# soedinglab/metaeuk

Hardware: AMD Instinct MI355X
Metric: prefilter+align ORF-fragments/sec (hits UNVERIFIED in this run: no CPU reference digest) (higher is better)
Workload: dtype packed i16 / i32 DP on u8 residues, i8 scores

## Files before the change

metaeuk_amd/csrc/mk_align.hip:

```cpp
#include "mk_align.hpp"
#include "mk_filters.hpp"
#include "mk_kernels.hpp"
#include "mk_segsort.hpp"
#include <algorithm>
#include <cmath>
#include <cstdlib>
#include <cstring>
#include <atomic>
#include <map>
#include <mutex>
#include <omp.h>

namespace mk {

namespace {

constexpr uint32_t KEY_CLS = 4096;
constexpr int SW_NBINCFG = SW_NCFG + 2;
constexpr uint32_t N_BINS = (uint32_t) SW_NBINCFG * KEY_CLS;
static_assert(SW_NCFG <= 16, "the bounds arrays keep 16 slots per kind");

__device__ __forceinline__ uint32_t len_class(uint32_t tLen) { return KEY_CLS - 1 - min(tLen >> 4, KEY_CLS - 1); }
__device__ __forceinline__ uint32_t sort_key(uint32_t qLen, uint32_t tLen) { return (uint32_t) sw_cfg_of(qLen) * KEY_CLS + len_class(tLen); }

// ... 461 lines not shown
        for (size_t k = 0; k < lens.size(); k++)
            if (!cached[k]) (*rowCache)[lens[k]].assign(&t.evalue[k * t.smax], &t.evalue[k * t.smax] + t.smax);
    if (t.bitScore.empty()) {
        t.bitScore.resize(32768);
        for (int s = 0; s < 32768; s++) t.bitScore[s] = static_cast<int>(ev.bitScore((double) s) + 0.5);
    }
}

void build_gate_table(const Evaluer &ev, double evalThr, const std::vector<uint64_t> &qOff, std::vector<GateEntry> &table, const AssembleTables *T) {
    uint32_t maxLen = 0;
    const size_t n = qOff.size() - 1;
    for (size_t i = 0; i < n; i++) maxLen = std::max<uint32_t>(maxLen, (uint32_t) (qOff[i + 1] - qOff[i]));
    std::vector<uint8_t> present(maxLen + 1, 0);
    for (size_t i = 0; i < n; i++) present[qOff[i + 1] - qOff[i]] = 1;
    table.assign(maxLen + 1, GateEntry{1 << 30, {0, 0, 0, 0, 0, 0, 0, 0}});
#pragma omp parallel for schedule(dynamic, 16)
    for (uint32_t L = 1; L <= maxLen; L++) {
        if (!present[L]) continue;
        GateEntry g;
        std::memset(&g, 0, sizeof(g));
        const int SCAN = 4096;
        const double *row = (T && L < T->lenIdx.size() && T->lenIdx[L] >= 0) ? T->evalue.data() + (size_t) T->lenIdx[L] * T->smax : nullptr;
        const auto eval = [&](int s) { return (row && (uint32_t) s < T->smax) ? row[s] : ev.evalue((double) s, (double) L); };
        int lastFail = 0;
        for (int s = SCAN; s >= 1; s--) {
            const bool pass = !(eval(s) > evalThr);
            if (!pass) { lastFail = s; break; }
        }
        g.s0 = lastFail >= SCAN ? (1 << 30) : lastFail + 1;
        for (int s = 1; s < 256 && s < g.s0; s++)
            if (!(eval(s) > evalThr)) g.mask[s >> 5] |= 1u << (s & 31);
        table[L] = g;
    }
}

#define ACHK(x) do { hipError_t e_ = (x); if (e_ != hipSuccess) { err = std::string(#x) + ": " + hipGetErrorString(e_); return MK_ERR_DEVICE; } } while (0)
#define ANULL(p) do { if (!(p)) { err = "device scratch allocation failed (" #p ")"; return MK_ERR_DEVICE; } } while (0)

static int device_scan(const uint32_t *in, uint32_t n, uint32_t *out, uint32_t *total, hipStream_t stream, std::string &err) {
    if (n == 0) { if (total) ACHK(hipMemsetAsync(total, 0, 4, stream)); return MK_OK; }
    const uint32_t nb = (n + SCAN_TILE - 1u) / SCAN_TILE;
    uint32_t *sums = (uint32_t *) dev_scratch("align_scansums", (size_t) nb * 4);
    ANULL(sums);
    hipLaunchKernelGGL(scan_sums_kernel, dim3(nb), dim3(256), 0, stream, in, n, sums);
    hipLaunchKernelGGL(scan_apply_kernel, dim3(nb), dim3(256), 0, stream, in, n, out, (const uint32_t *) sums, total);
    ACHK(hipGetLastError());
    return MK_OK;
}

struct AlignShapes {
    int cus = 256;
    uint32_t persistentBlocks[SW_NCFG];
    uint32_t unitsPerBlock = 0;
    int knownForce = -1, knownWaves = 12;
    bool fwdLargeFirst = false;
    bool multiLargeFirst = true;
    bool multiPrio = true;
    uint32_t multiPerCu[3] = {24, 12, 12};
};
static bool sw_early_exit() { return knob_long("MK_SW_EARLY_EXIT", 1) != 0; }
static const AlignShapes &align_shapes() {
    static AlignShapes S;
    static std::once_flag once;
    std::call_once(once, [] {
        int dev = 0;
        (void) hipGetDevice(&dev);
        if (hipDeviceGetAttribute(&S.cus, hipDeviceAttributeMultiprocessorCount, dev) != hipSuccess || S.cus <= 0) S.cus = 256;
        int perCu[SW_NCFG];
        for (int c = 0; c < SW_NCFG; c++) perCu[c] = 12;
        if (const char *e = knob("MK_SW_WAVES_PER_CU")) {
            int k = 0, last = 16;
            for (const char *p = e; *p && k < SW_NCFG; k++) {
                last = std::max(1, atoi(p));
                perCu[k] = last;
                while (*p && *p != ',') p++;
                if (*p == ',') p++;
            }
            for (; k < SW_NCFG; k++) perCu[k] = last;
        }
        for (int c = 0; c < SW_NCFG; c++) S.persistentBlocks[c] = (uint32_t) (S.cus * perCu[c]);
        S.unitsPerBlock = (uint32_t) std::max(0L, knob_long("MK_SW_UNITS_PER_BLOCK", 0));
        S.knownForce = (int) knob_long("MK_SW_KNOWN", -1);
        S.knownWaves = (int) std::max(1L, knob_long("MK_SW_KNOWN_WAVES", 12));
        S.multiPrio = knob_long("MK_SW_MULTI_PRIO", 1) != 0;
        S.fwdLargeFirst = knob_long("MK_SW_FWD_LARGE_FIRST", 0) != 0;
        S.multiLargeFirst = knob_long("MK_SW_MULTI_LARGE_FIRST", 1) != 0;
        if (const char *e = knob("MK_SW_MULTI_WAVES")) {
            int k = 0;
            for (const char *p = e; *p && k < 3; k++) { S.multiPerCu[k] = (uint32_t) std::max(1, atoi(p)); while (*p && *p != ',') p++; if (*p == ',') p++; }
        }
    });
    return S;
}

static int tpos_first_cfg(const AlignView &V) {
    static_assert(SW_NCFG == 11, "configurations 8 / 9 = 512 / 768 rows");
    if (!V.q_prof || knob_long("MK_SW_TPOS", 1) == 0 || knob_long("MK_SW_MULTI", 0) != 0 || knob_long("MK_SW_NARROW", -1) == 0) return -1;
    return 8;
}

static int run_sorted_sw(const AlignView &V, const mk_params &P, const SwJob *jobs, SwOut *out, const uint32_t *keys, uint32_t *hist, uint32_t *order,
                         uint32_t n, const char *tag, hipStream_t stream, std::string &err,
                         timed_begin_fn tb, timed_end_fn te, int *handles ,
                         const int32_t *knownScore ) {
    if (handles) for (int c = 0; c < SW_NCFG; c++) handles[c] = -1;
    if (n == 0) return MK_OK;
    const AlignShapes &S = align_shapes();
    uint32_t *dCursor = (uint32_t *) dev_scratch("align_bincursor", (size_t) N_BINS * 4);
    uint32_t *dBounds = (uint32_t *) dev_scratch("align_bounds", 64 * sizeof(uint32_t));
    uint32_t *hb = (uint32_t *) pinned_scratch("align_bounds_h", 64 * sizeof(uint32_t));
    ANULL(dCursor); ANULL(dBounds); ANULL(hb);
    int th = tb("align_sort", 12.0 * n, 0);
    hipLaunchKernelGGL(bin_scan_kernel, dim3(1), dim3(BIN_THREADS), 0, stream, hist, dCursor, dBounds);
    hipLaunchKernelGGL(bin_scatter_kernel, dim3((n + 255) / 256), dim3(256), 0, stream, keys, n, dCursor, order);
    te(th);
    ACHK(hipGetLastError());
    const bool knownPreferred = knownScore && !V.q_prof && (S.knownForce >= 0 ? S.knownForce != 0 : !V.co_resident);
    const bool multiLaunch = knob_long("MK_SW_MULTI", 0) != 0;
    if (multiLaunch && !knownPreferred && V.max_q_len <= (uint32_t) sw_cfg_rows(SW_NCFG - 1)) {
        uint32_t *dCnt = (uint32_t *) dev_scratch("align_multicounters", 64);
        ANULL(dCnt);
        ACHK(hipMemsetAsync(dCnt, 0, 64, stream));
        SwLaunch L;
        L.q_res = V.q_res; L.q_bias8 = V.q_bias8; L.q_prof = V.q_prof; L.t_res = V.t_res; L.mat = V.mat_aln;
        L.jobs = jobs; L.out = out; L.n_jobs = n; L.order = order;
        L.boundary = nullptr; L.boundary_stride = 0; L.boundary_job0 = 0;
        L.wave_start = nullptr; L.n_waves = 0; L.work_counter = nullptr; L.persistent_blocks = 0; L.units_per_block = 0;
        L.known_score = sw_early_exit() ? knownScore : nullptr;
        L.gap_open = P.gap_open; L.gap_extend = P.gap_extend;
        static const char *clsName[3] = {"rows32_64", "rows96_256", "rows384_1024"};
        static const int clsFirst[3] = {0, 3, 7};
        for (int kk = 0; kk < 3; kk++) {
            const int k = S.multiLargeFirst ? 2 - kk : kk;
            char nm[64];
            snprintf(nm, sizeof(nm), "%s_%s", tag, clsName[k]);
            th = tb(nm, 0, 0);
            if (handles) handles[clsFirst[k]] = th;
            const uint32_t units = (n + 3u) / 4u + (uint32_t) SW_NCFG;
            ACHK(launch_sw_multi(L, dBounds, dCnt + k, k, std::min(units, (uint32_t) S.cus * S.multiPerCu[k]), stream, S.multiPrio));
            te(th);
        }
        return MK_OK;
    }
    ACHK(hipMemcpyAsync(hb, dBounds, 64 * sizeof(uint32_t), hipMemcpyDeviceToHost, stream));
    ACHK(sync_wait(stream, "wait_align"));
    for (int c = 0; c < SW_NCFG; c++) {
        const uint32_t lo = hb[c], hi = hb[c + 1];
        if (hi <= lo) continue;
        SwLaunch L;
        L.q_res = V.q_res; L.q_bias8 = V.q_bias8; L.q_prof = V.q_prof; L.t_res = V.t_res; L.mat = V.mat_aln;
        L.jobs = jobs; L.out = out; L.n_jobs = hi - lo; L.order = order + lo;
        L.boundary = nullptr; L.boundary_stride = 0; L.boundary_job0 = 0;
        L.wave_start = nullptr; L.n_waves = 0; L.work_counter = nullptr; L.persistent_blocks = 0; L.units_per_block = 0; L.known_score = nullptr;
        L.gap_open = P.gap_open; L.gap_extend = P.gap_extend;
        if (c == SW_NCFG - 1 && V.max_q_len > (uint32_t) sw_cfg_rows(c)) {
            const uint32_t cls = KEY_CLS - 1 - (hb[32 + c] % KEY_CLS);
            const uint32_t stride = std::min<uint32_t>(V.max_t_len, (cls + 1) * 16);
            L.boundary = (uint32_t *) dev_scratch("align_border", (size_t) (hi - lo) * stride * sizeof(uint32_t));
            ANULL(L.boundary);
            L.boundary_stride = stride;
        }
        char nm[64];
        snprintf(nm, sizeof(nm), "%s_rows%d", tag, sw_cfg_rows(c));
        th = tb(nm, 0, 0);
        if (handles) handles[c] = th;
        if (knownScore && sw_cfg_known(c) && !V.q_prof && (S.knownForce >= 0 ? S.knownForce != 0 : !V.co_resident)) {
            uint32_t *dWork = (uint32_t *) dev_scratch("align_knowncounters", 64 * sizeof(uint32_t));
            ANULL(dWork);
            uint32_t *counter = dWork + (strcmp(tag, "sw_rev") == 0 ? 16 : 0) + c;
            ACHK(hipMemsetAsync(counter, 0, sizeof(uint32_t), stream));
            L.known_score = knownScore; L.work_counter = counter;
            L.persistent_blocks = (uint32_t) S.cus * (uint32_t) (sw_cfg_rows(c) <= 32 ? S.knownWaves : std::max(1, S.knownWaves / 2));
            ACHK(launch_sw_known(L, c, stream));
        } else {
            if (sw_early_exit()) L.known_score = knownScore;
            ACHK(launch_sw(L, c, stream));
        }
        te(th);
    }
    for (int pc = 0; pc < SW_NBINCFG - SW_NCFG; pc++) {
        const uint32_t lo = hb[SW_NCFG + pc], hi = hb[SW_NCFG + pc + 1];
        if (hi <= lo) continue;
        if (!knownScore || !V.q_prof) { err = "transposed position jobs without a known score"; return MK_ERR_DEVICE; }
        SwLaunch L;
        L.q_res = V.q_res; L.q_bias8 = V.q_bias8; L.q_prof = V.q_prof; L.t_res = V.t_res; L.mat = V.mat_aln;
        L.jobs = jobs; L.out = out; L.n_jobs = hi - lo; L.order = order + lo;
        L.boundary = nullptr; L.boundary_stride = 0; L.boundary_job0 = 0;
        L.wave_start = nullptr; L.n_waves = 0; L.work_counter = nullptr; L.persistent_blocks = 0; L.units_per_block = 0; L.known_score = knownScore;
        L.gap_open = P.gap_open; L.gap_extend = P.gap_extend;
        const int rows = sw_cfg_rows(8 + pc);
        char nm[64];
        snprintf(nm, sizeof(nm), "%s_rows%dt", tag, rows);
        th = tb(nm, 0, 0);
        ACHK(launch_sw_tpos(L, rows, (uint32_t) S.cus * (uint32_t) std::max(1L, knob_long("MK_SW_TPOS_WAVES", 32)), stream));
        te(th);
    }
    return MK_OK;
}

static int run_shared_fwd(const AlignView &V, const mk_params &P, const uint64_t *dHitOff, const mk_hit *dHits, const SwJob *jobs, SwOut *out,
                          uint32_t n, hipStream_t stream, std::string &err, timed_begin_fn tb, timed_end_fn te, int *handles ) {
    for (int c = 0; c < SW_NCFG; c++) handles[c] = -1;
    if (n == 0) return MK_OK;
    const AlignShapes &S = align_shapes();
    const uint32_t nq = V.n_queries;
    const uint32_t nb = (nq + PLAN_BLOCK - 1u) / PLAN_BLOCK;
    const uint32_t maxRuns = n / ORDER_TILE + nq + 1;
    uint32_t *dOrder = (uint32_t *) dev_scratch("align_order", (size_t) n * 4);
    uint32_t *dWave = (uint32_t *) dev_scratch("align_wavestart", ((size_t) n + 1) * 4);
    uint32_t *dPlan = (uint32_t *) dev_scratch("align_plan", ((size_t) nq * 2 + (size_t) maxRuns * 2 + (size_t) nb * (PLAN_NV + 1)) * 4);
    uint32_t *dBounds = (uint32_t *) dev_scratch("align_bounds", 64 * sizeof(uint32_t));
    uint32_t *hb = (uint32_t *) pinned_scratch("align_bounds_h", 64 * sizeof(uint32_t));
    uint32_t *dWork = (uint32_t *) dev_scratch("align_workcounters", 256);
    ANULL(dOrder); ANULL(dWave); ANULL(dPlan); ANULL(dBounds); ANULL(hb); ANULL(dWork);
    ACHK(hipMemsetAsync(dWork, 0, 256, stream));
    const long narrowForce = knob_long("MK_SW_NARROW", -1);
    const bool narrow = narrowForce >= 0 ? narrowForce != 0 : V.q_prof != nullptr;
    PlanArgs A;
    A.hitOff = dHitOff; A.q_off = V.q_off; A.nq = nq; A.nPairs = n; A.narrow = narrow;
    A.jobOff = dPlan; A.waveOff = dPlan + nq; A.runQuery = dPlan + 2 * (size_t) nq; A.runIndex = A.runQuery + maxRuns; A.blockSums = A.runIndex + maxRuns;
    A.bounds = dBounds; A.waveStart = dWave;
    int th = tb("align_sort", 24.0 * n, 0);
    hipLaunchKernelGGL(plan_sums_kernel, dim3(nb), dim3(PLAN_BLOCK), 0, stream, A);
    hipLaunchKernelGGL(plan_offsets_kernel, dim3(nb), dim3(PLAN_BLOCK), 0, stream, A);
    ACHK(hipGetLastError());
    ACHK(hipMemcpyAsync(hb, dBounds, 64 * sizeof(uint32_t), hipMemcpyDeviceToHost, stream));
// ... 407 lines not shown
```

metaeuk_amd/csrc/mk_kernels.hpp:

```cpp
#pragma once
#include <hip/hip_runtime.h>
#include <cstdint>

namespace mk {

struct SwJob {
    uint64_t t_start;
    uint32_t q_start;
    uint32_t q_len;
    uint32_t t_len;
    int32_t q_step;
    int32_t t_step;
    uint32_t slot;
};
struct SwOut { int32_t score; int32_t end_col; int32_t end_row; int32_t pad; };

struct SwLaunch {
    const uint8_t *q_res; const int8_t *q_bias8;
    const int8_t *q_prof = nullptr;
    const uint8_t *t_res;
    const int8_t *mat;
    const SwJob *jobs; SwOut *out; uint64_t n_jobs;
    const uint32_t *order;
    uint32_t *boundary;
    uint32_t boundary_stride;
    int gap_open, gap_extend;
    const uint32_t *wave_start; uint64_t n_waves;
    uint32_t *work_counter;
    uint32_t *work_counter_t = nullptr;
    uint32_t t_max_rows = 0;
    uint32_t persistent_blocks;
    uint32_t units_per_block;
    uint64_t boundary_job0;
    const int32_t *known_score;
    bool narrow = false;
};

constexpr int SW_NCFG = 11;
__host__ __device__ inline int sw_cfg_rows(int c) {
    const int rows[SW_NCFG] = {32, 48, 64, 96, 128, 192, 256, 384, 512, 768, 1024};
    return rows[c];
}
__host__ __device__ inline bool sw_cfg_packed(int c) { return sw_cfg_rows(c) <= 768; }
__host__ __device__ inline uint32_t sw_cfg_jobs_per_wave(int c, bool narrow = false) {
    const int rows = sw_cfg_rows(c);
    return rows <= 256 ? 8u : (rows <= 768 ? (narrow ? 8u : 4u) : 1u);
}
__host__ __device__ inline int sw_cfg_of(uint32_t qLen) {
    int c = 0;
    while (c < SW_NCFG - 1 && (uint32_t) sw_cfg_rows(c) < qLen) c++;
    return c;
}
hipError_t launch_sw(const SwLaunch &L, int cfg, hipStream_t stream);
hipError_t launch_sw_score(const SwLaunch &L, int cfg, hipStream_t stream);
__host__ __device__ inline bool sw_cfg_known(int c) { return sw_cfg_rows(c) <= 64; }
hipError_t launch_sw_known(const SwLaunch &L, int cfg, hipStream_t stream);
constexpr uint32_t SW_TPOS_MAX_ROWS = 256;
hipError_t launch_sw_tpos(const SwLaunch &L, int rows, uint32_t blocksPerClass, hipStream_t stream);
hipError_t launch_sw_multi(const SwLaunch &L, const uint32_t *bounds, uint32_t *counter, int cls, uint32_t blocks, hipStream_t stream, bool prio = true);

template <class ScoreFn>
__host__ __device__ inline int ungapped_on_diagonal_fn(ScoreFn score_of, uint32_t qLen, const uint8_t *t, uint32_t tLen,
                                                       int diagonal, uint32_t minDist) {
    uint32_t len = 0, q0 = 0, t0 = 0;
    if (diagonal >= 0 && minDist < qLen) { len = tLen < qLen - minDist ? tLen : qLen - minDist; q0 = minDist; }
    else if (diagonal < 0 && minDist < tLen) { len = tLen - minDist < qLen ? tLen - minDist : qLen; t0 = minDist; }
    int score = 0, best = 0;
    for (uint32_t k = 0; k < len; k++) {
        const int curr = score_of(q0 + k, (uint32_t) t[t0 + k]);
        score = score + curr > 0 ? score + curr : 0;
        best = best > score ? best : score;
    }
    return best;
}
template <class ScoreFn>
__host__ __device__ inline int ungapped_score_fn(ScoreFn score_of, uint32_t qLen, const uint8_t *t, uint32_t tLen, uint32_t d16) {
    if (qLen >= 32768u || tLen >= 32768u) {
        int best = 0;
        for (uint32_t d = 1; d <= 1u + tLen / 32768u; d++) {
            const int real = (int) (0u - d * 65536u + d16);
            const int m = ungapped_on_diagonal_fn(score_of, qLen, t, tLen, real, (uint32_t) (real < 0 ? -real : real));
            best = best > m ? best : m;
        }
        for (uint32_t d = 0; d <= qLen / 65536u; d++) {
            const int real = (int) (d * 65536u + d16);
            const int m = ungapped_on_diagonal_fn(score_of, qLen, t, tLen, real, (uint32_t) (real < 0 ? -real : real));
            best = best > m ? best : m;
        }
        return best;
    }
    const uint32_t dist = ((0x10000u - d16) & 0xFFFFu) < d16 ? ((0x10000u - d16) & 0xFFFFu) : d16;
    return ungapped_on_diagonal_fn(score_of, qLen, t, tLen, (int) (short) (uint16_t) d16, dist);
}
template <typename MatT>
__host__ __device__ inline int ungapped_score(const MatT *smat, const uint8_t *q, const int8_t *corr, uint32_t qLen, const uint8_t *t, uint32_t tLen, uint32_t d16) {
    return ungapped_score_fn([=](uint32_t i, uint32_t tr) -> int { return (int) (int8_t) ((int8_t) smat[q[i] * 21 + tr] + corr[i]); }, qLen, t, tLen, d16);
}
__host__ __device__ inline int ungapped_score_profile(const int8_t *aln, uint32_t qLen, const uint8_t *t, uint32_t tLen, uint32_t d16) {
    return ungapped_score_fn([=](uint32_t i, uint32_t tr) -> int { return (int) aln[(size_t) i * 32 + tr]; }, qLen, t, tLen, d16);
}

struct UngappedJob { uint64_t t_start; uint32_t q_start; uint32_t q_len; uint32_t t_len; uint32_t diagonal; };
struct UngappedLaunch {
    const uint8_t *q_res; const int8_t *q_corr;
    const uint8_t *t_masked;
    const int8_t *mat;
    const UngappedJob *jobs; int32_t *out; uint64_t n_jobs;
};
hipError_t launch_ungapped(const UngappedLaunch &L, hipStream_t stream);
// ... 36 lines not shown
```

metaeuk_amd/csrc/mk_sw.hip:

```cpp
#include "mk_kernels.hpp"
#include <algorithm>
#include <mutex>

namespace mk {

template <int G>
__device__ __forceinline__ uint32_t shift_up(uint32_t top, uint32_t x, int laneInGroup) {
    if constexpr (G == 16) {
        return (uint32_t) __builtin_amdgcn_update_dpp((int) top, (int) x, 0x111 , 0xf, 0xf, false);
    } else if constexpr (G == 64) {
        return (uint32_t) __builtin_amdgcn_update_dpp((int) top, (int) x, 0x138 , 0xf, 0xf, false);
    } else {
        const uint32_t v = (uint32_t) __builtin_amdgcn_update_dpp((int) top, (int) x, 0x138 , 0xf, 0xf, false);
        return laneInGroup == 0 ? top : v;
    }
}

template <int G>
__device__ __forceinline__ uint32_t shift_up_zero(uint32_t x, int laneInGroup) {
    if constexpr (G == 16) return (uint32_t) __builtin_amdgcn_update_dpp((int) x, (int) x, 0x111 , 0xf, 0xf, true);
    else return shift_up<G>(0u, x, laneInGroup);
}

__device__ __forceinline__ int max3i(int a, int b, int c) { return max(max(a, b), c); }
// ... 71 lines not shown
                const int q = row0 + row;
                const bool real = q < qLen;
                const int64_t qi = (int64_t) profQStart + (int64_t) (real ? q : 0) * profQStep;
                sQ[row] = real ? L.q_res[qi] : (uint8_t) 255;
                sB[row] = real ? L.q_bias8[qi] : (int8_t) 0;
            }
            __builtin_amdgcn_fence(__ATOMIC_ACQ_REL, "wavefront");
            __builtin_amdgcn_wave_barrier();
            for (int idx = SHARED ? (int) threadIdx.x : lane; idx < 22 * ROWS; idx += SHARED ? BLOCK : G) {
                const int t = idx / ROWS, row = idx - t * ROWS;
                const uint32_t qc = sQ[row];
                prof[idx] = (t < 21 && qc != 255u) ? (int8_t) ((int) sMat[t * 21 + (int) qc] + (int) sB[row]) : (int8_t) 0;
            }
        }
        __builtin_amdgcn_fence(__ATOMIC_ACQ_REL, "wavefront");
        __builtin_amdgcn_wave_barrier();

        int H[R], E[R];
        uint32_t key[R];
#pragma unroll
        for (int r = 0; r < R; r++) { H[r] = 0; E[r] = 0; key[r] = 0; }
        uint32_t out0 = 0, out1 = 21u;
        int hupPrev = 0;
        const int steps = tLen > 0 ? tLen + G - 1 : 0;
        const bool readTop = (tile > 0);
        const bool writeBottom = (tile + 1 < nTiles);
        const int laneRow = (int) (threadIdx.x & 15u);
        const int64_t tBase = (int64_t) job.t_start;
        const int64_t tStep = (int64_t) job.t_step;
        const int tLast = max(tLen - 1, 0);
        uint32_t tq0 = L.t_res[tBase + (int64_t) min(laneRow, tLast) * tStep], tq1 = L.t_res[tBase + (int64_t) min(16 + laneRow, tLast) * tStep],
                 tq2 = L.t_res[tBase + (int64_t) min(32 + laneRow, tLast) * tStep];
        for (int s0 = 0; s0 < steps; s0 += 16) {
            uint32_t tcur = tq0;
            tq0 = tq1; tq1 = tq2;
            tq2 = L.t_res[tBase + (int64_t) min(s0 + 48 + laneRow, tLast) * tStep];
            const int sEnd = min(s0 + 16, steps);
            for (int s = s0; s < sEnd; s++) {
                uint32_t top0 = 0;
                const uint32_t top1 = s < tLen ? tcur : 21u;
                tcur = (uint32_t) __builtin_amdgcn_update_dpp(0, (int) tcur, 0x12F , 0xf, 0xf, false);
                if (readTop && lane == 0 && s < tLen) top0 = border[s];
                const uint32_t in0 = shift_up<G>(top0, out0, lane);
                const uint32_t tres = shift_up<G>(top1, out1, lane);
                const int hup = (int) (in0 & 0xFFFFu);
                int F = (int) (in0 >> 16);
                const int c = s - lane;
                const uint32_t cinv = 0x1FFFFu - (uint32_t) max(c, 0);
                int sc[R];
                load_scores<R>(prof + tres * ROWS + lane * R, sc);
                int dsave = hupPrev;
#pragma unroll
                for (int r = 0; r < R; r++) {
                    const int d = min(dsave + sc[r], 32767);
                    dsave = H[r];
                    const int h = max3i(d, E[r], F);
                    key[r] = max(key[r], ((uint32_t) h << 17) | cinv);
                    const int ho = h - go;
                    E[r] = max3i(E[r] - ge, ho, 0);
                    F = max3i(F - ge, ho, 0);
                    H[r] = h;
                }
                hupPrev = hup;
                out0 = (uint32_t) H[R - 1] | ((uint32_t) F << 16);
                out1 = tres;
                if (writeBottom && lane == G - 1 && c >= 0 && c < tLen) border[c] = out0;
            }
            if constexpr (!SHARED) {
                if (known > 0) {
                    bool seen = false;
#pragma unroll
                    for (int r = 0; r < R; r++) seen |= (key[r] >> 17) == (uint32_t) known;
                    const unsigned long long m = __ballot(seen);
                    const unsigned long long mine = G == 64 ? ~0ull : ((1ull << (G & 63)) - 1ull) << (((unsigned) threadIdx.x & 63u) / G * G);
                    if ((m & mine) != 0ull && ++after > NEED) break;
                }
            }
        }
#pragma unroll
        for (int r = 0; r < R; r++) {
            if (key[r] > bestKey) { bestKey = key[r]; bestRow = row0 + lane * R + r; }
        }
        __builtin_amdgcn_fence(__ATOMIC_ACQ_REL, "wavefront");
        __builtin_amdgcn_wave_barrier();
    }
#pragma unroll
    for (int m = G / 2; m >= 1; m >>= 1) {
        const uint32_t ok = (uint32_t) __shfl_xor((int) bestKey, m, G);
        const int orow = __shfl_xor(bestRow, m, G);
        if (ok > bestKey || (ok == bestKey && orow < bestRow)) { bestKey = ok; bestRow = orow; }
    }
    if (have && lane == 0) {
        SwOut o;
        o.score = (int32_t) (bestKey >> 17);
        o.end_col = o.score > 0 ? (int32_t) (0x1FFFFu - (bestKey & 0x1FFFFu)) : -1;
        o.end_row = o.score > 0 ? bestRow : -1;
        o.pad = 0;
        L.out[job.slot] = o;
    }
}

#ifndef MK_HELPER_PRIO
#define MK_HELPER_PRIO 3
#endif
template <int G, int R, int BLOCK, bool SHARED>
__global__ __launch_bounds__(BLOCK) void sw_kernel(SwLaunch L) {
    if (!SHARED && MK_HELPER_PRIO) __builtin_amdgcn_s_setprio(MK_HELPER_PRIO);
// ... 467 lines not shown
#pragma unroll
                    for (int k = 0; k < RP / 4; k++) {
                        const uint64_t xa = qa[k], xb = qb[k];
                        wa[2 * k] = (uint32_t) xa; wa[2 * k + 1] = (uint32_t) (xa >> 32); wb[2 * k] = (uint32_t) xb; wb[2 * k + 1] = (uint32_t) (xb >> 32);
                    }
                } else {
#pragma unroll
                for (int k = 0; k < RP / 2; k++) { wa[k] = reinterpret_cast<const uint32_t *>(pa)[k]; wb[k] = reinterpret_cast<const uint32_t *>(pb)[k]; }
                }
                pk16 dsave = hupPrev;
#pragma unroll
                for (int r = 0; r < R; r++) {
                    const pk16 sc = pk_from(__builtin_amdgcn_perm(wb[r / 2], wa[r / 2], (r & 1) ? 0x07060302u : 0x05040100u));
                    const pk16 d = SAT ? __builtin_elementwise_add_sat(dsave, sc) : dsave + sc;
                    dsave = H[r];
                    const pk16 h = pk_max(pk_max(d, E[r]), F);
                    best = pk_max(best, h);
                    const pk16 ho = pk_subs0(h, go2);
                    E[r] = pk_max(pk_subs0(E[r], ge2), ho);
                    F = pk_max(pk_subs0(F, ge2), ho);
                    H[r] = h;
                }
                hupPrev = hup;
                outH = pk_bits(H[R - 1]);
                outF = pk_bits(F);
                outRes = tres;
            }
            const uint32_t rose = pk_bits(best) ^ bestIn;
            if (rose & 0xFFFFu) roseA = s0;
            if (rose >> 16) roseB = s0;
        }
        uint32_t b = pk_bits(best);
#pragma unroll
        for (int m = G / 2; m >= 1; m >>= 1) b = pk_bits(pk_max(pk_from(b), pk_from((uint32_t) __shfl_xor((int) b, m, G))));
        uint32_t cA = (pk_bits(best) & 0xFFFFu) == (b & 0xFFFFu) ? (uint32_t) max(roseA + 15 - lane, 0) : 0x7FFFFFFFu;
        uint32_t cB = (pk_bits(best) >> 16) == (b >> 16) ? (uint32_t) max(roseB + 15 - lane, 0) : 0x7FFFFFFFu;
#pragma unroll
        for (int m = G / 2; m >= 1; m >>= 1) {
            cA = min(cA, (uint32_t) __shfl_xor((int) cA, m, G));
            cB = min(cB, (uint32_t) __shfl_xor((int) cB, m, G));
        }
        if (lane == 0) {
            SwOut o;
            o.end_row = -1; o.pad = 0;
            if (haveA) { o.score = (int32_t) (int16_t) (b & 0xFFFFu); o.end_col = (int32_t) min(cA, (uint32_t) lastA); L.out[jobA.slot] = o; }
            if (haveB) { o.score = (int32_t) (int16_t) (b >> 16); o.end_col = (int32_t) min(cB, (uint32_t) lastB); L.out[jobB.slot] = o; }
        }
        __builtin_amdgcn_fence(__ATOMIC_ACQ_REL, "wavefront");
        __builtin_amdgcn_wave_barrier();
        }
    }
}

template <int R, int RP>
__global__ __launch_bounds__(64) void swq_kernel(SwLaunch L) {
    constexpr int G = 16, ROWS = G * RP, NDP = 8;
    static_assert(RP >= R && RP % 2 == 0 && G * R * 127 <= 32767, "small tiles only");
    extern __shared__ __attribute__((aligned(16))) int8_t smem[];
    int16_t *prof = reinterpret_cast<int16_t *>(smem);
    constexpr int PROF1 = 22 * ROWS;
    int8_t *sMat = smem + (size_t) NDP * PROF1 * sizeof(int16_t);
    uint8_t *sQ = reinterpret_cast<uint8_t *>(sMat + 448);
    int8_t *sB = reinterpret_cast<int8_t *>(sQ + NDP * ROWS);
    for (int k = (int) threadIdx.x; k < 441; k += 64) sMat[k] = L.mat[k];
    const int lane = threadIdx.x % G, grp = threadIdx.x / G;
    const pk16 go2 = pk_splat(L.gap_open), ge2 = pk_splat(L.gap_extend), zero2 = pk_splat(0);
    const uint64_t nUnits = (L.n_jobs + NDP - 1) / NDP;
    for (;;) {
        uint32_t u = 0;
        if (threadIdx.x == 0) u = atomicAdd(L.work_counter, 1u);
        u = (uint32_t) __builtin_amdgcn_readfirstlane((int) u);
        if ((uint64_t) u >= nUnits) break;
        const uint64_t j0 = (uint64_t) u * NDP;
        const uint64_t ja = j0 + 2 * grp, jb = ja + 1;
        const bool haveA = ja < L.n_jobs, haveB = jb < L.n_jobs;
        const SwJob jobA = L.jobs[L.order[haveA ? ja : j0]], jobB = L.jobs[L.order[haveB ? jb : j0]];
        const int tLenA = haveA ? (int) jobA.t_len : 0, tLenB = haveB ? (int) jobB.t_len : 0;
        const uint32_t SA = haveA ? (uint32_t) L.known_score[jobA.slot] & 0xFFFFu : 0xFFFFu, SB = haveB ? (uint32_t) L.known_score[jobB.slot] & 0xFFFFu : 0xFFFFu;
        const uint32_t S2 = SA | (SB << 16);
        for (int i = (int) threadIdx.x; i < NDP * ROWS; i += 64) {
            const int dp = i / ROWS, slot = i - dp * ROWS;
            const uint64_t j = j0 + (uint64_t) dp;
            uint8_t qc = 255; int8_t bc = 0;
            if (j < L.n_jobs) {
                const SwJob jj = L.jobs[L.order[j]];
                const int row = RP == R ? slot : (slot / RP) * R + slot % RP;
                if (row < (int) jj.q_len && (RP == R || slot % RP < R)) {
                    const int64_t qi = (int64_t) jj.q_start + (int64_t) row * jj.q_step;
                    qc = L.q_res[qi]; bc = L.q_bias8[qi];
                }
            }
            sQ[i] = qc; sB[i] = bc;
        }
        __builtin_amdgcn_fence(__ATOMIC_ACQ_REL, "wavefront");
        __builtin_amdgcn_wave_barrier();
        for (int i = (int) threadIdx.x; i < NDP * PROF1; i += 64) {
            const int dp = i / PROF1, rem = i - dp * PROF1, t = rem / ROWS, slot = rem - t * ROWS;
            const uint32_t qc = sQ[dp * ROWS + slot];
            prof[i] = (t < 21 && qc != 255u) ? (int16_t) ((int) sMat[t * 21 + (int) qc] + (int) sB[dp * ROWS + slot]) : (int16_t) 0;
        }
        __builtin_amdgcn_fence(__ATOMIC_ACQ_REL, "wavefront");
        __builtin_amdgcn_wave_barrier();

        pk16 H[R], E[R];
#pragma unroll
        for (int r = 0; r < R; r++) { H[r] = zero2; E[r] = zero2; }
        pk16 best = zero2, hupPrev = zero2;
        constexpr uint32_t ROWB = (uint32_t) ROWS * 2u, NOCOL = 21u * ROWB | (21u * ROWB) << 16;
        uint32_t outH = 0, outF = 0, outRes = NOCOL;
        const int tMax = max(tLenA, tLenB);
        const int steps = tMax > 0 ? (tMax + G - 1 + 15) & ~15 : 0;
        const int laneRow = lane & 15;
        const int lastA = max(tLenA - 1, 0), lastB = max(tLenB - 1, 0);
        const int64_t baseA = (int64_t) jobA.t_start, baseB = (int64_t) jobB.t_start, stepA = jobA.t_step, stepB = jobB.t_step;
        const auto fetch = [&](int col) -> uint32_t {
            const uint32_t ra = col < tLenA ? (uint32_t) L.t_res[baseA + (int64_t) min(col, lastA) * stepA] : 21u;
            const uint32_t rb = col < tLenB ? (uint32_t) L.t_res[baseB + (int64_t) min(col, lastB) * stepB] : 21u;
            return ra * ROWB | (rb * ROWB) << 16;
        };
        const char *profA = reinterpret_cast<const char *>(prof + (size_t) (2 * grp) * PROF1 + lane * RP);
        const char *profB = reinterpret_cast<const char *>(prof + (size_t) (2 * grp + 1) * PROF1 + lane * RP);
        uint32_t foundA = 0xFFFFFFFFu, foundB = 0xFFFFFFFFu;
        uint32_t closed2 = 0u;
        uint32_t tq0 = fetch(laneRow), tq1 = fetch(16 + laneRow), tq2 = fetch(32 + laneRow);
        for (int s0 = 0; s0 < steps; s0 += 16) {
            uint32_t tcur = tq0;
            tq0 = tq1; tq1 = tq2;
            tq2 = fetch(s0 + 48 + laneRow);
#pragma unroll
            for (int k = 0; k < 16; k++) {
                const uint32_t top = tcur;
                tcur = (uint32_t) __builtin_amdgcn_update_dpp(0, (int) tcur, 0x12F , 0xf, 0xf, false);
                const pk16 hup = pk_from(shift_up_zero<G>(outH, lane));
                pk16 F = pk_from(shift_up_zero<G>(outF, lane));
                const uint32_t tres = shift_up<G>(top, outRes, lane);
                const int16_t *pa = reinterpret_cast<const int16_t *>(profA + (tres & 0xFFFFu)), *pb = reinterpret_cast<const int16_t *>(profB + (tres >> 16));
                uint32_t wa[RP / 2], wb[RP / 2];
#pragma unroll
                for (int kk = 0; kk < RP / 2; kk++) { wa[kk] = reinterpret_cast<const uint32_t *>(pa)[kk]; wb[kk] = reinterpret_cast<const uint32_t *>(pb)[kk]; }
                pk16 dsave = hupPrev;
#pragma unroll
                for (int r = 0; r < R; r++) {
                    const pk16 sc = pk_from(__builtin_amdgcn_perm(wb[r / 2], wa[r / 2], (r & 1) ? 0x07060302u : 0x05040100u));
                    const pk16 d = dsave + sc;
                    dsave = H[r];
                    const pk16 h = pk_max(pk_max(d, E[r]), F);
                    best = pk_max(best, h);
                    const pk16 ho = pk_subs0(h, go2);
                    E[r] = pk_max(pk_subs0(E[r], ge2), ho);
                    F = pk_max(pk_subs0(F, ge2), ho);
                    H[r] = h;
                }
                hupPrev = hup;
                outH = pk_bits(H[R - 1]);
                outF = pk_bits(F);
                outRes = tres;
                const uint32_t x = (pk_bits(best) ^ S2) | closed2;
                const uint32_t hit = (x - 0x00010001u) & ~x & 0x80008000u;
                if (__builtin_amdgcn_ballot_w64(hit != 0u) != 0ull) {
                    const int c = s0 + k - lane;
                    if ((x & 0xFFFFu) == 0u) {
                        int row = 0;
#pragma unroll
                        for (int r = R - 1; r >= 0; r--) if ((pk_bits(H[r]) & 0xFFFFu) == SA) row = r;
                        foundA = ((uint32_t) c << 12) | (uint32_t) (lane * R + row);
                        closed2 |= 0x1u;
                    }
                    if ((x >> 16) == 0u) {
                        int row = 0;
#pragma unroll
                        for (int r = R - 1; r >= 0; r--) if ((pk_bits(H[r]) >> 16) == SB) row = r;
                        foundB = ((uint32_t) c << 12) | (uint32_t) (lane * R + row);
                        closed2 |= 0x10000u;
                    }
                }
            }
        }
#pragma unroll
        for (int m = G / 2; m >= 1; m >>= 1) {
            foundA = min(foundA, (uint32_t) __shfl_xor((int) foundA, m, G));
            foundB = min(foundB, (uint32_t) __shfl_xor((int) foundB, m, G));
        }
        if (lane == 0) {
            SwOut o;
            o.pad = 0;
            if (haveA) { const bool ok = foundA != 0xFFFFFFFFu; o.score = ok ? (int32_t) SA : 0; o.end_col = ok ? (int32_t) (foundA >> 12) : -1; o.end_row = ok ? (int32_t) (foundA & 0xFFFu) : -1; L.out[jobA.slot] = o; }
            if (haveB) { const bool ok = foundB != 0xFFFFFFFFu; o.score = ok ? (int32_t) SB : 0; o.end_col = ok ? (int32_t) (foundB >> 12) : -1; o.end_row = ok ? (int32_t) (foundB & 0xFFFu) : -1; L.out[jobB.slot] = o; }
        }
        __builtin_amdgcn_fence(__ATOMIC_ACQ_REL, "wavefront");
        __builtin_amdgcn_wave_barrier();
    }
}

hipError_t launch_sw_known(const SwLaunch &L, int cfg, hipStream_t stream) {
    if (!L.order || !L.work_counter || !L.known_score || cfg < 0 || cfg >= SW_NCFG || !sw_cfg_known(cfg)) return hipErrorInvalidValue;
    if (L.n_jobs == 0) return hipSuccess;
    const uint64_t nUnits = (L.n_jobs + 7) / 8;
    const uint64_t grid = std::min<uint64_t>(nUnits, L.persistent_blocks ? L.persistent_blocks : nUnits);
    const int rows = sw_cfg_rows(cfg);
    const size_t prows = rows == 48 ? 64 : rows;
    const size_t lds = (size_t) 8 * 22 * prows * sizeof(int16_t) + 448 + 2 * 8 * prows;
    switch (rows) {
        case 32: hipLaunchKernelGGL((swq_kernel<2, 2>), dim3((unsigned) grid), dim3(64), lds, stream, L); break;
        case 48: hipLaunchKernelGGL((swq_kernel<3, 4>), dim3((unsigned) grid), dim3(64), lds, stream, L); break;
        case 64: hipLaunchKernelGGL((swq_kernel<4, 4>), dim3((unsigned) grid), dim3(64), lds, stream, L); break;
        default: return hipErrorInvalidValue;
    }
    return hipGetLastError();
}

hipError_t launch_sw_score(const SwLaunch &L, int cfg, hipStream_t stream) {
    if (!L.wave_start || !L.work_counter || !L.order || cfg < 0 || cfg >= SW_NCFG || !sw_cfg_packed(cfg)) return hipErrorInvalidValue;
    if (L.n_waves == 0) return hipSuccess;
    const uint64_t grid = L.units_per_block ? (L.n_waves + L.units_per_block - 1) / L.units_per_block
                                            : std::min<uint64_t>(L.n_waves, L.persistent_blocks ? L.persistent_blocks : L.n_waves);
    const int rows = sw_cfg_rows(cfg);
    const size_t prows = rows == 48 ? 64 : rows;
    const size_t lds = (size_t) 22 * prows * sizeof(int16_t) + 448 + 2 * prows;
    if (L.t_max_rows) {
        if (!L.work_counter_t || !L.q_prof || !L.narrow || L.t_max_rows > SWT_MAX_ROWS) return hipErrorInvalidValue;
        hipLaunchKernelGGL(swt_kernel<0>, dim3((unsigned) grid), dim3(64), swt_image_bytes(rows), stream, L);
        if (L.t_max_rows > 64u) hipLaunchKernelGGL(swt_kernel<1>, dim3((unsigned) grid), dim3(64), swt_image_bytes(rows), stream, L);
        if (L.t_max_rows > 128u) hipLaunchKernelGGL(swt_kernel<2>, dim3((unsigned) grid), dim3(64), swt_image_bytes(rows), stream, L);
    }
    switch (rows) {
        case 32: hipLaunchKernelGGL((swp_kernel<2>), dim3((unsigned) grid), dim3(64), lds, stream, L); break;
        case 48: hipLaunchKernelGGL((swp_kernel<3, 4>), dim3((unsigned) grid), dim3(64), lds, stream, L); break;
        case 64: hipLaunchKernelGGL((swp_kernel<4>), dim3((unsigned) grid), dim3(64), lds, stream, L); break;
        case 96: hipLaunchKernelGGL((swp_kernel<6>), dim3((unsigned) grid), dim3(64), lds, stream, L); break;
        case 128: hipLaunchKernelGGL((swp_kernel<8>), dim3((unsigned) grid), dim3(64), lds, stream, L); break;
        case 192: hipLaunchKernelGGL((swp_kernel<12>), dim3((unsigned) grid), dim3(64), lds, stream, L); break;
        case 256: hipLaunchKernelGGL((swp_kernel<16>), dim3((unsigned) grid), dim3(64), lds, stream, L); break;
        case 384: if (L.narrow) hipLaunchKernelGGL((swp_kernel<24, 24, 16>), dim3((unsigned) grid), dim3(64), lds, stream, L);
                  else hipLaunchKernelGGL((swp_kernel<12, 12, 32>), dim3((unsigned) grid), dim3(64), lds, stream, L);
                  break;
        case 512: hipLaunchKernelGGL((swp_kernel<16, 16, 32>), dim3((unsigned) grid), dim3(64), lds, stream, L); break;
        case 768: hipLaunchKernelGGL((swp_kernel<24, 24, 32>), dim3((unsigned) grid), dim3(64), lds, stream, L); break;
        default: return hipErrorInvalidValue;
    }
    return hipGetLastError();
}

hipError_t launch_sw_tpos(const SwLaunch &L, int rows, uint32_t blocksPerClass, hipStream_t stream) {
    if (!L.q_prof || !L.order || !L.known_score || rows <= 0) return hipErrorInvalidValue;
    if (L.n_jobs == 0) return hipSuccess;
    const unsigned grid = (unsigned) std::min<uint64_t>((L.n_jobs + 7) / 8, std::max<uint32_t>(1u, blocksPerClass));
    hipLaunchKernelGGL(swtp_kernel<0>, dim3(grid), dim3(64), swt_image_bytes(rows), stream, L);
    hipLaunchKernelGGL(swtp_kernel<1>, dim3(grid), dim3(64), swt_image_bytes(rows), stream, L);
    hipLaunchKernelGGL(swtp_kernel<2>, dim3(grid), dim3(64), swt_image_bytes(rows), stream, L);
    return hipGetLastError();
}

template <int G, int R, int BLOCK>
static hipError_t launch_one(const SwLaunch &L, hipStream_t stream) {
    if (L.wave_start) {
        const size_t lds = (size_t) 24 * G * R;
        if (L.n_waves == 0) return hipSuccess;
        const uint64_t grid = L.units_per_block ? (L.n_waves + L.units_per_block - 1) / L.units_per_block
                                                : std::min<uint64_t>(L.n_waves, L.persistent_blocks ? L.persistent_blocks : L.n_waves);
// ... 59 lines not shown
```

Baseline: 2.525 million.

## Use int8 query profiles and early exit in known-score SW kernel, extend to 128 rows

The known-score packed SW kernel gains an int8 profile mode, now the default. Profiles are built with byte-wise SIMD adds and perm shuffles from a transposed, biased substitution matrix, which halves LDS footprint and profile reads per column. The kernel also exits a tile early once both jobs have found their known end cell, controlled by a new early_exit flag. It is extended to 96- and 128-row configurations. A redundant saturation clamp in the main SW kernel is removed when it cannot overflow, and the known-path selection logic is refactored into a helper. The risks are the extra unpack work per cell and the correctness of the byte-bias trick.

New measurement: 2.537 million (median of 4 runs). No clear change (+0.5%).

```diff
diff --git a/metaeuk_amd/csrc/mk_align.hip b/metaeuk_amd/csrc/mk_align.hip
--- a/metaeuk_amd/csrc/mk_align.hip
+++ b/metaeuk_amd/csrc/mk_align.hip
@@ -537,13 +537,19 @@
     int cus = 256;
     uint32_t persistentBlocks[SW_NCFG];
     uint32_t unitsPerBlock = 0;
-    int knownForce = -1, knownWaves = 12;
+    int knownWaves = 12;
     bool fwdLargeFirst = false;
     bool multiLargeFirst = true;
     bool multiPrio = true;
     uint32_t multiPerCu[3] = {24, 12, 12};
 };
 static bool sw_early_exit() { return knob_long("MK_SW_EARLY_EXIT", 1) != 0; }
+constexpr bool SW_KNOWN_CO_RESIDENT = false;
+static bool sw_known_preferred(const AlignView &V) {
+    if (V.q_prof) return false;
+    const long force = knob_long("MK_SW_KNOWN", -1);
+    return force >= 0 ? force != 0 : (!V.co_resident || SW_KNOWN_CO_RESIDENT);
+}
 static const AlignShapes &align_shapes() {
     static AlignShapes S;
     static std::once_flag once;
@@ -565,7 +571,6 @@
         }
         for (int c = 0; c < SW_NCFG; c++) S.persistentBlocks[c] = (uint32_t) (S.cus * perCu[c]);
         S.unitsPerBlock = (uint32_t) std::max(0L, knob_long("MK_SW_UNITS_PER_BLOCK", 0));
-        S.knownForce = (int) knob_long("MK_SW_KNOWN", -1);
         S.knownWaves = (int) std::max(1L, knob_long("MK_SW_KNOWN_WAVES", 12));
         S.multiPrio = knob_long("MK_SW_MULTI_PRIO", 1) != 0;
         S.fwdLargeFirst = knob_long("MK_SW_FWD_LARGE_FIRST", 0) != 0;
@@ -600,7 +605,7 @@
     hipLaunchKernelGGL(bin_scatter_kernel, dim3((n + 255) / 256), dim3(256), 0, stream, keys, n, dCursor, order);
     te(th);
     ACHK(hipGetLastError());
-    const bool knownPreferred = knownScore && !V.q_prof && (S.knownForce >= 0 ? S.knownForce != 0 : !V.co_resident);
+    const bool knownPreferred = knownScore && sw_known_preferred(V);
     const bool multiLaunch = knob_long("MK_SW_MULTI", 0) != 0;
     if (multiLaunch && !knownPreferred && V.max_q_len <= (uint32_t) sw_cfg_rows(SW_NCFG - 1)) {
         uint32_t *dCnt = (uint32_t *) dev_scratch("align_multicounters", 64);
@@ -649,14 +654,15 @@
         snprintf(nm, sizeof(nm), "%s_rows%d", tag, sw_cfg_rows(c));
         th = tb(nm, 0, 0);
         if (handles) handles[c] = th;
-        if (knownScore && sw_cfg_known(c) && !V.q_prof && (S.knownForce >= 0 ? S.knownForce != 0 : !V.co_resident)) {
+        if (knownPreferred && sw_cfg_known(c)) {
             uint32_t *dWork = (uint32_t *) dev_scratch("align_knowncounters", 64 * sizeof(uint32_t));
             ANULL(dWork);
             uint32_t *counter = dWork + (strcmp(tag, "sw_rev") == 0 ? 16 : 0) + c;
             ACHK(hipMemsetAsync(counter, 0, sizeof(uint32_t), stream));
-            L.known_score = knownScore; L.work_counter = counter;
-            L.persistent_blocks = (uint32_t) S.cus * (uint32_t) (sw_cfg_rows(c) <= 32 ? S.knownWaves : std::max(1, S.knownWaves / 2));
-            ACHK(launch_sw_known(L, c, stream));
+            L.known_score = knownScore; L.work_counter = counter; L.early_exit = sw_early_exit();
+            const int rows = sw_cfg_rows(c);
+            L.persistent_blocks = (uint32_t) S.cus * (uint32_t) std::max(1, rows <= 32 ? S.knownWaves : S.knownWaves / 2);
+            ACHK(launch_sw_known(L, c, stream, knob_long("MK_SW_KNOWN_PROF", 8) == 16 ? 16 : 8));
         } else {
             if (sw_early_exit()) L.known_score = knownScore;
             ACHK(launch_sw(L, c, stream));
diff --git a/metaeuk_amd/csrc/mk_kernels.hpp b/metaeuk_amd/csrc/mk_kernels.hpp
--- a/metaeuk_amd/csrc/mk_kernels.hpp
+++ b/metaeuk_amd/csrc/mk_kernels.hpp
@@ -33,6 +33,7 @@
     uint32_t units_per_block;
     uint64_t boundary_job0;
     const int32_t *known_score;
+    bool early_exit = true;
     bool narrow = false;
 };
 
@@ -53,8 +54,9 @@
 }
 hipError_t launch_sw(const SwLaunch &L, int cfg, hipStream_t stream);
 hipError_t launch_sw_score(const SwLaunch &L, int cfg, hipStream_t stream);
-__host__ __device__ inline bool sw_cfg_known(int c) { return sw_cfg_rows(c) <= 64; }
-hipError_t launch_sw_known(const SwLaunch &L, int cfg, hipStream_t stream);
+__host__ __device__ inline bool sw_cfg_known(int c) { return sw_cfg_rows(c) <= 128; }
+size_t sw_known_lds_bytes(int cfg, int profBits = 8);
+hipError_t launch_sw_known(const SwLaunch &L, int cfg, hipStream_t stream, int profBits = 8);
 constexpr uint32_t SW_TPOS_MAX_ROWS = 256;
 hipError_t launch_sw_tpos(const SwLaunch &L, int rows, uint32_t blocksPerClass, hipStream_t stream);
 hipError_t launch_sw_multi(const SwLaunch &L, const uint32_t *bounds, uint32_t *counter, int cls, uint32_t blocks, hipStream_t stream, bool prio = true);
diff --git a/metaeuk_amd/csrc/mk_sw.hip b/metaeuk_amd/csrc/mk_sw.hip
--- a/metaeuk_amd/csrc/mk_sw.hip
+++ b/metaeuk_amd/csrc/mk_sw.hip
@@ -147,7 +147,8 @@
                 int dsave = hupPrev;
 #pragma unroll
                 for (int r = 0; r < R; r++) {
-                    const int d = min(dsave + sc[r], 32767);
+                    int d = dsave + sc[r];
+                    if constexpr (G * R * 127 > 32767) d = min(d, 32767);
                     dsave = H[r];
                     const int h = max3i(d, E[r], F);
                     key[r] = max(key[r], ((uint32_t) h << 17) | cinv);
@@ -721,17 +722,30 @@
     }
 }
 
-template <int R, int RP>
+__device__ __forceinline__ uint32_t add_bytes(uint32_t x, uint32_t y) {
+    return ((x & 0x7F7F7F7Fu) + (y & 0x7F7F7F7Fu)) ^ ((x ^ y) & 0x80808080u);
+}
+template <int R, int RP, bool P8>
 __global__ __launch_bounds__(64) void swq_kernel(SwLaunch L) {
+    if (MK_HELPER_PRIO) __builtin_amdgcn_s_setprio(MK_HELPER_PRIO);
     constexpr int G = 16, ROWS = G * RP, NDP = 8;
     static_assert(RP >= R && RP % 2 == 0 && G * R * 127 <= 32767, "small tiles only");
+    static_assert(!P8 || RP == 2 || RP == 4 || RP == 8, "int8 profiles: a lane's bytes of a column are one aligned word");
     extern __shared__ __attribute__((aligned(16))) int8_t smem[];
+    constexpr int ESZ = P8 ? 1 : 2;
+    constexpr int PROF1 = 22 * ROWS;
     int16_t *prof = reinterpret_cast<int16_t *>(smem);
-    constexpr int PROF1 = 22 * ROWS;
-    int8_t *sMat = smem + (size_t) NDP * PROF1 * sizeof(int16_t);
+    int8_t *sMat = smem + (size_t) NDP * PROF1 * ESZ;
     uint8_t *sQ = reinterpret_cast<uint8_t *>(sMat + 448);
     int8_t *sB = reinterpret_cast<int8_t *>(sQ + NDP * ROWS);
-    for (int k = (int) threadIdx.x; k < 441; k += 64) sMat[k] = L.mat[k];
+    if constexpr (P8) {
+        for (int k = (int) threadIdx.x; k < 22 * 24; k += 64) {
+            const int q = k / 24, t = k - q * 24;
+            sMat[k] = (int8_t) ((q < 21 && t < 21) ? ((uint8_t) L.mat[t * 21 + q] ^ 0x80u) : 0x80u);
+        }
+    } else {
+        for (int k = (int) threadIdx.x; k < 441; k += 64) sMat[k] = L.mat[k];
+    }
     const int lane = threadIdx.x % G, grp = threadIdx.x / G;
     const pk16 go2 = pk_splat(L.gap_open), ge2 = pk_splat(L.gap_extend), zero2 = pk_splat(0);
     const uint64_t nUnits = (L.n_jobs + NDP - 1) / NDP;
@@ -747,6 +761,45 @@
         const int tLenA = haveA ? (int) jobA.t_len : 0, tLenB = haveB ? (int) jobB.t_len : 0;
         const uint32_t SA = haveA ? (uint32_t) L.known_score[jobA.slot] & 0xFFFFu : 0xFFFFu, SB = haveB ? (uint32_t) L.known_score[jobB.slot] & 0xFFFFu : 0xFFFFu;
         const uint32_t S2 = SA | (SB << 16);
+        if constexpr (P8) {
+        __builtin_amdgcn_fence(__ATOMIC_ACQ_REL, "wavefront");
+        __builtin_amdgcn_wave_barrier();
+        constexpr int CH = ROWS / 4;
+        uint32_t *prof32 = reinterpret_cast<uint32_t *>(smem);
+#pragma unroll 1
+        for (int i = (int) threadIdx.x; i < NDP * CH; i += 64) {
+            const int dp = i / CH, ch = i - dp * CH;
+            const uint64_t j = j0 + (uint64_t) dp;
+            const bool hj = j < L.n_jobs;
+            const SwJob jj = L.jobs[L.order[hj ? j : j0]];
+            uint32_t x[4][6];
+#pragma unroll
+            for (int k = 0; k < 4; k++) {
+                const int slot = ch * 4 + k;
+                const int row = RP == R ? slot : (slot / RP) * R + slot % RP;
+                const bool real = hj && row < (int) jj.q_len && (RP == R || slot % RP < R);
+                const int64_t qi = (int64_t) jj.q_start + (int64_t) (real ? row : 0) * jj.q_step;
+                const uint32_t qc = real ? min((uint32_t) L.q_res[qi], 21u) : 21u;
+                const uint32_t yb = real ? (uint32_t) (uint8_t) L.q_bias8[qi] * 0x01010101u : 0u;
+                const uint32_t *m = reinterpret_cast<const uint32_t *>(sMat + qc * 24);
+#pragma unroll
+                for (int w = 0; w < 6; w++) x[k][w] = add_bytes(m[w], qc < 21u ? yb : 0u);
+            }
+#pragma unroll
+            for (int w = 0; w < 6; w++) {
+                const uint32_t a0 = __builtin_amdgcn_perm(x[1][w], x[0][w], 0x05010400u), a1 = __builtin_amdgcn_perm(x[1][w], x[0][w], 0x07030602u);
+                const uint32_t b0 = __builtin_amdgcn_perm(x[3][w], x[2][w], 0x05010400u), b1 = __builtin_amdgcn_perm(x[3][w], x[2][w], 0x07030602u);
+                const uint32_t y[4] = {__builtin_amdgcn_perm(b0, a0, 0x05040100u), __builtin_amdgcn_perm(b0, a0, 0x07060302u),
+                                       __builtin_amdgcn_perm(b1, a1, 0x05040100u), __builtin_amdgcn_perm(b1, a1, 0x07060302u)};
+#pragma unroll
+                for (int tt = 0; tt < 4; tt++) {
+                    const int t = 4 * w + tt;
+                    if (t < 21) prof32[(dp * PROF1 + t * ROWS) / 4 + ch] = y[tt] ^ 0x80008000u;
+                    else if (t == 21) prof32[(dp * PROF1 + t * ROWS) / 4 + ch] = 0x00800080u;
+                }
+            }
+        }
+        } else {
         for (int i = (int) threadIdx.x; i < NDP * ROWS; i += 64) {
             const int dp = i / ROWS, slot = i - dp * ROWS;
             const uint64_t j = j0 + (uint64_t) dp;
@@ -768,6 +821,7 @@
             const uint32_t qc = sQ[dp * ROWS + slot];
             prof[i] = (t < 21 && qc != 255u) ? (int16_t) ((int) sMat[t * 21 + (int) qc] + (int) sB[dp * ROWS + slot]) : (int16_t) 0;
         }
+        }
         __builtin_amdgcn_fence(__ATOMIC_ACQ_REL, "wavefront");
         __builtin_amdgcn_wave_barrier();
 
@@ -775,7 +829,7 @@
 #pragma unroll
         for (int r = 0; r < R; r++) { H[r] = zero2; E[r] = zero2; }
         pk16 best = zero2, hupPrev = zero2;
-        constexpr uint32_t ROWB = (uint32_t) ROWS * 2u, NOCOL = 21u * ROWB | (21u * ROWB) << 16;
+        constexpr uint32_t ROWB = (uint32_t) (ROWS * ESZ), NOCOL = 21u * ROWB | (21u * ROWB) << 16;
         uint32_t outH = 0, outF = 0, outRes = NOCOL;
         const int tMax = max(tLenA, tLenB);
         const int steps = tMax > 0 ? (tMax + G - 1 + 15) & ~15 : 0;
@@ -787,10 +841,13 @@
             const uint32_t rb = col < tLenB ? (uint32_t) L.t_res[baseB + (int64_t) min(col, lastB) * stepB] : 21u;
             return ra * ROWB | (rb * ROWB) << 16;
         };
-        const char *profA = reinterpret_cast<const char *>(prof + (size_t) (2 * grp) * PROF1 + lane * RP);
-        const char *profB = reinterpret_cast<const char *>(prof + (size_t) (2 * grp + 1) * PROF1 + lane * RP);
+        const char *profA = reinterpret_cast<const char *>(smem) + ((size_t) (2 * grp) * PROF1 + lane * RP) * ESZ;
+        const char *profB = reinterpret_cast<const char *>(smem) + ((size_t) (2 * grp + 1) * PROF1 + lane * RP) * ESZ;
         uint32_t foundA = 0xFFFFFFFFu, foundB = 0xFFFFFFFFu;
         uint32_t closed2 = 0u;
+        const unsigned long long mine = 0xFFFFull << (((unsigned) threadIdx.x & 63u) / G * G);
+        const bool earlyExit = L.early_exit;
+        int after = 0;
         uint32_t tq0 = fetch(laneRow), tq1 = fetch(16 + laneRow), tq2 = fetch(32 + laneRow);
         for (int s0 = 0; s0 < steps; s0 += 16) {
             uint32_t tcur = tq0;
@@ -803,14 +860,30 @@
                 const pk16 hup = pk_from(shift_up_zero<G>(outH, lane));
                 pk16 F = pk_from(shift_up_zero<G>(outF, lane));
                 const uint32_t tres = shift_up<G>(top, outRes, lane);
-                const int16_t *pa = reinterpret_cast<const int16_t *>(profA + (tres & 0xFFFFu)), *pb = reinterpret_cast<const int16_t *>(profB + (tres >> 16));
-                uint32_t wa[RP / 2], wb[RP / 2];
-#pragma unroll
-                for (int kk = 0; kk < RP / 2; kk++) { wa[kk] = reinterpret_cast<const uint32_t *>(pa)[kk]; wb[kk] = reinterpret_cast<const uint32_t *>(pb)[kk]; }
+                const char *pa = profA + (tres & 0xFFFFu), *pb = profB + (tres >> 16);
+                constexpr int NW = P8 ? (RP + 3) / 4 : RP / 2;
+                uint32_t wa[NW], wb[NW];
+                if constexpr (P8 && RP == 2) {
+                    wa[0] = *reinterpret_cast<const uint16_t *>(pa); wb[0] = *reinterpret_cast<const uint16_t *>(pb);
+                } else if constexpr (P8 && RP == 8) {
+                    const uint64_t xa = *reinterpret_cast<const uint64_t *>(__builtin_assume_aligned(pa, 8)), xb = *reinterpret_cast<const uint64_t *>(__builtin_assume_aligned(pb, 8));
+                    wa[0] = (uint32_t) xa; wa[1] = (uint32_t) (xa >> 32); wb[0] = (uint32_t) xb; wb[1] = (uint32_t) (xb >> 32);
+                } else {
+#pragma unroll
+                    for (int kk = 0; kk < NW; kk++) { wa[kk] = reinterpret_cast<const uint32_t *>(pa)[kk]; wb[kk] = reinterpret_cast<const uint32_t *>(pb)[kk]; }
+                }
                 pk16 dsave = hupPrev;
 #pragma unroll
                 for (int r = 0; r < R; r++) {
-                    const pk16 sc = pk_from(__builtin_amdgcn_perm(wb[r / 2], wa[r / 2], (r & 1) ? 0x07060302u : 0x05040100u));
+                    pk16 sc;
+                    if constexpr (P8) {
+                        const uint32_t b = (uint32_t) (r & 3);
+                        const uint32_t sel =(r & 1) ? ((10u + b / 2u) << 24 | (4u + b) << 16 | (8u + b / 2u) << 8 | b) : (0x0C000C00u | (4u + b) << 16 | b);
+                        const uint32_t v = __builtin_amdgcn_perm(wb[r / 4], wa[r / 4], sel);
+                        sc = (r & 1) ? pk_from(v) : pk_from(v) - pk_splat(128);
+                    } else {
+                        sc = pk_from(__builtin_amdgcn_perm(wb[r / 2], wa[r / 2], (r & 1) ? 0x07060302u : 0x05040100u));
+                    }
                     const pk16 d = dsave + sc;
                     dsave = H[r];
                     const pk16 h = pk_max(pk_max(d, E[r]), F);
@@ -844,6 +917,10 @@
                     }
                 }
             }
+            if (earlyExit) {
+                const unsigned long long mA = __builtin_amdgcn_ballot_w64((closed2 & 0xFFFFu) != 0u), mB = __builtin_amdgcn_ballot_w64((closed2 >> 16) != 0u);
+                if (((mA & mine) != 0ull || !haveA) && ((mB & mine) != 0ull || !haveB) && ++after > 1) break;
+            }
         }
 #pragma unroll
         for (int m = G / 2; m >= 1; m >>= 1) {
@@ -861,19 +938,38 @@
     }
 }
 
-hipError_t launch_sw_known(const SwLaunch &L, int cfg, hipStream_t stream) {
-    if (!L.order || !L.work_counter || !L.known_score || cfg < 0 || cfg >= SW_NCFG || !sw_cfg_known(cfg)) return hipErrorInvalidValue;
+static size_t sw_known_slots(int rows, bool p8) { return rows == 48 ? 64 : (rows == 96 && p8 ? 128 : (size_t) rows); }
+size_t sw_known_lds_bytes(int cfg, int profBits) {
+    const size_t prows = sw_known_slots(sw_cfg_rows(cfg), profBits == 8);
+    return profBits == 8 ? (size_t) 8 * 22 * prows + 22 * 24
+                         : (size_t) 8 * 22 * prows * sizeof(int16_t) + 448 + 2 * 8 * prows;
+}
+
+hipError_t launch_sw_known(const SwLaunch &L, int cfg, hipStream_t stream, int profBits) {
+    if (!L.order || !L.work_counter || !L.known_score || cfg < 0 || cfg >= SW_NCFG || !sw_cfg_known(cfg) || (profBits != 8 && profBits != 16)) return hipErrorInvalidValue;
     if (L.n_jobs == 0) return hipSuccess;
     const uint64_t nUnits = (L.n_jobs + 7) / 8;
     const uint64_t grid = std::min<uint64_t>(nUnits, L.persistent_blocks ? L.persistent_blocks : nUnits);
     const int rows = sw_cfg_rows(cfg);
-    const size_t prows = rows == 48 ? 64 : rows;
-    const size_t lds = (size_t) 8 * 22 * prows * sizeof(int16_t) + 448 + 2 * 8 * prows;
-    switch (rows) {
-        case 32: hipLaunchKernelGGL((swq_kernel<2, 2>), dim3((unsigned) grid), dim3(64), lds, stream, L); break;
-        case 48: hipLaunchKernelGGL((swq_kernel<3, 4>), dim3((unsigned) grid), dim3(64), lds, stream, L); break;
-        case 64: hipLaunchKernelGGL((swq_kernel<4, 4>), dim3((unsigned) grid), dim3(64), lds, stream, L); break;
-        default: return hipErrorInvalidValue;
+    const size_t lds = sw_known_lds_bytes(cfg, profBits);
+    if (profBits == 8) {
+        switch (rows) {
+            case 32: hipLaunchKernelGGL((swq_kernel<2, 2, true>), dim3((unsigned) grid), dim3(64), lds, stream, L); break;
+            case 48: hipLaunchKernelGGL((swq_kernel<3, 4, true>), dim3((unsigned) grid), dim3(64), lds, stream, L); break;
+            case 64: hipLaunchKernelGGL((swq_kernel<4, 4, true>), dim3((unsigned) grid), dim3(64), lds, stream, L); break;
+            case 96: hipLaunchKernelGGL((swq_kernel<6, 8, true>), dim3((unsigned) grid), dim3(64), lds, stream, L); break;
+            case 128: hipLaunchKernelGGL((swq_kernel<8, 8, true>), dim3((unsigned) grid), dim3(64), lds, stream, L); break;
+            default: return hipErrorInvalidValue;
+        }
+    } else {
+        switch (rows) {
+            case 32: hipLaunchKernelGGL((swq_kernel<2, 2, false>), dim3((unsigned) grid), dim3(64), lds, stream, L); break;
+            case 48: hipLaunchKernelGGL((swq_kernel<3, 4, false>), dim3((unsigned) grid), dim3(64), lds, stream, L); break;
+            case 64: hipLaunchKernelGGL((swq_kernel<4, 4, false>), dim3((unsigned) grid), dim3(64), lds, stream, L); break;
+            case 96: hipLaunchKernelGGL((swq_kernel<6, 6, false>), dim3((unsigned) grid), dim3(64), lds, stream, L); break;
+            case 128: hipLaunchKernelGGL((swq_kernel<8, 8, false>), dim3((unsigned) grid), dim3(64), lds, stream, L); break;
+            default: return hipErrorInvalidValue;
+        }
     }
     return hipGetLastError();
 }
```
